# pratyushkumar211/industrial_nnmpc_2021

Measured on AMD Instinct MI355X. Metric: condensed-QP solves/sec (CDU offline datagen), higher is better.
Workload: dtype f64; 1 GPU; cdu_offline_data: synthetic CDU-size plant (n=4480 vars, m=8960 box rows, n_aug=284), 100000 sampled x0 per GPU per step, whole sequences u* written out; batch_per_gpu=100000, total_batch=100000, method=auto, parallelism=dp1 (sharded samples, 1 RCCL gather of the first moves pe...

## Files before the change

include/nnmpc.h:

```cpp
#ifndef NNMPC_H
#define NNMPC_H
#include <stdint.h>
#ifdef __cplusplus
extern "C" {
#endif

#define NNMPC_OK 0
#define NNMPC_EINVAL (-1)
#define NNMPC_EHIP (-2)
#define NNMPC_ENOMEM (-3)
#define NNMPC_ENOTIMPL (-4)

#define NNMPC_HOST 0
#define NNMPC_DEVICE 1

#define NNMPC_ST_OPTIMAL 0
#define NNMPC_ST_MAXITER 1
#define NNMPC_ST_NUMERIC 2

typedef struct nnmpc_qp nnmpc_qp;
typedef struct nnmpc_nn nnmpc_nn;

typedef struct {
  int32_t max_batch;
// ... 53 lines not shown
  double asm_predict_ms;
  double asm_predict_flops;
  int64_t asm_overlapped_passes;
  double mult_ms;
  int64_t mult_launches;
  double sens_ms;
  int64_t sens_launches;
  int64_t sens_lds_problems;
  int64_t sens_slab_problems;
  double sens_total_ms;
  double adj_ms;
  int64_t adj_launches;
  int64_t adj_lds_problems;
  int64_t adj_slab_problems;
  double adj_total_ms;
} nnmpc_qp_stats;

const char* nnmpc_last_error(void);

int nnmpc_qp_create(nnmpc_qp** out, int32_t n, int32_t nu, int32_t n_aug, const double* P,
                    const double* tq, const double* Kunc, const nnmpc_qp_opts* opts);
int nnmpc_qp_destroy(nnmpc_qp* h);

int nnmpc_qp_solve_batch(nnmpc_qp* h, int32_t B, const double* x0, const double* lb,
                         const double* ub, double* u, uint32_t* active, int32_t* status,
                         int32_t* iters, int32_t ptr_kind);

int nnmpc_qp_solve_batch_warm(nnmpc_qp* h, int32_t B, const double* x0, const double* lb,
                              const double* ub, const uint8_t* guess, double* u, uint32_t* active,
                              int32_t* status, int32_t* iters, int32_t ptr_kind);
// ... 214 lines not shown
```

industrial_nnmpc_2021_amd/_lib.py:

```python
import ctypes as C
import os

_HERE = os.path.dirname(os.path.abspath(__file__))
LIB_PATH = os.path.join(_HERE, "libnnmpc_hip.so")

HOST, DEVICE = 0, 1
ST_OPTIMAL, ST_MAXITER, ST_NUMERIC = 0, 1, 2
OUT_SEQUENCE, OUT_FIRST_MOVE = 0, 1
EINVAL, EHIP, ENOMEM, ENOTIMPL = -1, -2, -3, -4


class QpOpts(C.Structure):
    _fields_ = [("max_batch", C.c_int32), ("nb", C.c_int32), ("max_ipm_iters", C.c_int32),
                ("max_polish_rounds", C.c_int32), ("max_refine", C.c_int32),
                ("max_rounds", C.c_int32), ("sub_steps", C.c_int32), ("stale_max_changes", C.c_int32),
                ("stale_cg_limit", C.c_int32), ("method", C.c_int32), ("asm_max_active", C.c_int32),
                ("asm_max_rounds", C.c_int32), ("asm_f32_rounds", C.c_int32), ("seg_max", C.c_int32), ("asm_tail_batch", C.c_int32), ("asm_predict_iters", C.c_int32), ("asm_overlap", C.c_int32), ("ipm_tol", C.c_float), ("refine_tol", C.c_double),
                ("bound_tol", C.c_double)]


class QpStats(C.Structure):
    _fields_ = [("problems", C.c_int64), ("rounds", C.c_int64), ("factorizations", C.c_int64),
                ("ipm_iterations", C.c_int64), ("panel_launches", C.c_int64),
                ("panel_ms", C.c_double), ("diag_ms", C.c_double), ("trsv_ms", C.c_double),
                ("total_ms", C.c_double), ("panel_flops", C.c_double), ("trsv_solves", C.c_int64), ("asm_solved", C.c_int64),
                ("asm_rounds", C.c_int64), ("asm_gemm_launches", C.c_int64), ("asm_gemm_ms", C.c_double),
                ("asm_gemm_flops", C.c_double), ("asm_lambda_ms", C.c_double), ("asm_update_ms", C.c_double), ("asm_lambda_flops", C.c_double),
                ("asm_lambda_bytes", C.c_double), ("asm_e1max", C.c_double),
                ("asm_e2max", C.c_double), ("asm_full_checks", C.c_int64), ("asm_lambda32_ms", C.c_double),
                ("asm_lambda64_ms", C.c_double), ("asm_lambda32_flops", C.c_double),
                ("asm_lambda32_launches", C.c_int64), ("asm_lambda64_launches", C.c_int64), ("asm_far_passes", C.c_int64), ("asm_side_ms", C.c_double),
                ("asm_small_passes", C.c_int64), ("asm_predict_launches", C.c_int64), ("asm_predict_ms", C.c_double),
                ("asm_predict_flops", C.c_double), ("asm_overlapped_passes", C.c_int64),
                ("mult_ms", C.c_double), ("mult_launches", C.c_int64),
                ("sens_ms", C.c_double), ("sens_launches", C.c_int64), ("sens_lds_problems", C.c_int64),
                ("sens_slab_problems", C.c_int64), ("sens_total_ms", C.c_double),
                ("adj_ms", C.c_double), ("adj_launches", C.c_int64), ("adj_lds_problems", C.c_int64),
                ("adj_slab_problems", C.c_int64), ("adj_total_ms", C.c_double)]


CL_MPC, CL_NN, CL_SATDLQR, CL_US, CL_NN_UNSTD = 0, 1, 2, 3, 4
NN_STRUCTURED, NN_UNSTD, NN_UNSTD_RELU = 0, 1, 2
CL_PLANT_LINEAR, CL_PLANT_CSTRS_FLASH, CSTRS_NPAR = 0, 1, 51


class ClModel(C.Structure):
    _fields_ = [(k, C.c_int32) for k in ("nx", "nu", "ny", "nd", "nz")] + \
               [(k, C.c_void_p) for k in ("A", "B", "C", "Bp", "Aaug", "Baug", "Caug", "L", "tb", "Qb", "Qy", "q0", "Cd",
                                          "Eb", "Xb", "Xu", "Qaug", "Raug", "Maug", "ulb", "uub", "x0", "xhat0", "uprev0")]


class ClSlot(C.Structure):
    _fields_ = [("kind", C.c_int32), ("qp", C.c_void_p), ("nlayers", C.c_int32), ("dims", C.c_void_p), ("W", C.c_void_p),
# ... 308 lines not shown
```

industrial_nnmpc_2021_amd/csrc/qp_asm.h:

```cpp
#pragma once
#include <hip/hip_runtime.h>
#include <stdint.h>
#include <type_traits>

#if defined(ASM_WG_TU) && ASM_WG_TU >= 0
#define ASM_OWN_KERNELS 0
#else
#define ASM_OWN_KERNELS 1
#endif

namespace nnmpc {

constexpr int ASM_MLDS = 176;
constexpr int ASM_TS = 16 * 17;
enum { ASM_RUN = 0, ASM_DONE = 1, ASM_FALLBACK = 2, ASM_CERT = 3, ASM_WIDE = 4, ASM_INVALID = 5 };
constexpr int ASM_NBIN = 8;
constexpr int ASM_NREG = 6;
constexpr int ASM_NCNT = 40;
constexpr int ASM_CNT_KSUM = 0;
constexpr int ASM_CNT_SLAB = 1;
constexpr int ASM_CNT_ROWS64 = 2;
constexpr int ASM_CNT_LAST = 3;
constexpr int ASM_CNT_F64 = 4;
constexpr int ASM_CNT_F32 = 16;
// ... 5 lines not shown
constexpr int ASM_CNT_BIG64R = 31;
constexpr int ASM_CNT_BIG32B = 39;
constexpr double ASM_REFINE_TOL = 1e-12;
constexpr int ASM_GRACE = 10;
constexpr int ASM_CNT_WIDE = 12;
constexpr int ASM_CNT_WKSUM = 30;
constexpr int ASM_TAIL_MB = 8;
constexpr int ASM_CNT_TAIL = 35;
constexpr int ASM_CNT_FFTILES = 38;
constexpr int ASM_CNT_DONE = 14;
__host__ __device__ constexpr int asm_list_counter(int list) {
  return list < ASM_NBIN ? 4 + list : (list < ASM_NLIST ? ASM_CNT_F32 + list - ASM_NBIN : (list == ASM_NLIST ? ASM_CNT_BIG32 : (list == ASM_NLIST + 1 ? ASM_CNT_BIG64 : (list == ASM_NLIST + 2 ? ASM_CNT_BIG32B : ASM_CNT_BIG64R))));
}
__host__ __device__ constexpr int asm_list_of_counter(int c) { return c >= ASM_CNT_F32 ? ASM_NBIN + c - ASM_CNT_F32 : c - 4; }
constexpr int ASM_NKG = 3;
constexpr int ASM_NSCAN = ASM_NLIST + 9 + 2 * ASM_NKG;
constexpr int ASM_CNT_ROWS32 = 15;
__host__ __device__ constexpr int asm_bin_cap(int b) { return 16 * (b + 4); }

struct AsmDev {
  int n, np, nu, nseg;
  int max_active;
  int max_rounds;
  double bound_tol, stat_tol, pscale;
  double e1max, e2max;
  const double* x0;
  int ka;
  const double* Kunc;
  int pred_w;
  int pred_f64;
  int winit;
// ... 43 lines not shown
  unsigned char* redo;
  int* lrank;
  int* ctot;
  int use_f32;
  int W;
  int* rowprob;
  int wrows;
  unsigned char* wmark;
  const double* xhw;
  int tail_gi;
  int use_wg;
  int refine;
  double refine_tol;
  int refine_later;
  int early64;
  int* wflag;
  double* work;
  double* scratch;
  double* u_out;
  int ldu, nout;
  uint32_t* act_out;
  int* status_out;
  int* iters_out;
  int words;
};

__device__ __forceinline__ size_t tri(int i, int j) { return (size_t)i * (i + 1) / 2 + j; }

#if ASM_OWN_KERNELS
__global__ __launch_bounds__(256) void asm_init_k(AsmDev d, int nrows) {
// ... 15 lines not shown
      const double x = d.xunc[o + r];
      double lb = lbf, ub = ubf;
      if (!kfix) { const int k = r % d.nu; lb = d.lb[(size_t)p * d.nu + k]; ub = d.ub[(size_t)p * d.nu + k]; }
      s = x > ub ? 1 : (x < lb ? 2 : 0);
    }
    d.st[(size_t)p * d.n + r] = (unsigned char)s;
  }
  int invalid = 0;
  for (int k = lane; k < d.nu; k += 64) invalid |= !(d.lb[(size_t)p * d.nu + k] <= d.ub[(size_t)p * d.nu + k]);
  for (int k = lane; k < d.ka; k += 64) invalid |= !(fabs(d.x0[(size_t)p * d.ka + k]) <= 1.79e308);
  invalid = __any(invalid);
  if (lane == 0) {
    d.rounds[p] = 0; d.state[p] = invalid ? ASM_INVALID : ASM_RUN;
    d.prec[p] = (d.use_f32 && !d.guess && !(d.pred_w && d.pred_f64)) ? 0 : 1;
    d.redo[p] = 0;
    d.ninf_best[p] = 0x7fffffff; d.alpha[p] = ASM_GRACE;
    d.hi[p] = max(wi, d.guess ? 0 : d.pred_w);
  }
}
#endif

__device__ __forceinline__ int asm_count_one(const AsmDev& d, int p, int hi_p, int* wsum) {
  const int tid = threadIdx.x, lane = tid & 63, wave = tid >> 6;
  const unsigned char* st = d.st + (size_t)p * d.n;
  const bool words = (d.n & 3) == 0;
  const int hi = min(d.n, hi_p);
  const int nw = words ? (hi + 3) >> 2 : hi;
  const int per = (nw + 255) / 256;
  const int j0 = min(nw, tid * per), j1 = min(nw, j0 + per);
  const uint32_t* sw = reinterpret_cast<const uint32_t*>(st);
// ... 57 lines not shown
    int k = inc - c;
    if (words) {
      for (int j = j0; j < j1; ++j) {
        const uint32_t w = sw[j];
        if (w & 0xffu) idx[k++] = 4 * j;
        if (w & 0xff00u) idx[k++] = 4 * j + 1;
        if (w & 0xff0000u) idx[k++] = 4 * j + 2;
        if (w & 0xff000000u) idx[k++] = 4 * j + 3;
      }
    } else {
      for (int j = j0; j < j1; ++j) if (st[j]) idx[k++] = j;
    }
  }
  return m;
}
#if ASM_OWN_KERNELS
__global__ __launch_bounds__(256) void asm_count_k(AsmDev d) {
  const int p = blockIdx.x * 4 + (threadIdx.x >> 6);
  if (p >= d.nseg || d.state[p] != ASM_RUN) return;
  const int m = asm_count_wave(d, p, d.hi[p]);
  if ((threadIdx.x & 63) == 0) {
    d.mg[p] = m;
    if (m <= d.max_active && d.work) {
      const double md = (double)m;
      d.work[3 * p] += md * md * md / 3.0 + 2.0 * md * md;
      d.work[3 * p + 1] += 8.0 * (md * (md + 1.0) / 2.0 + 2.0 * md);
      if (d.prec[p] == 0 && m <= (d.use_wg ? ASM_BIG32B : ASM_BIG32)) d.work[3 * p + 2] += md * md * md / 3.0 + 2.0 * md * md;
    }
    if (m > d.max_active) d.state[p] = ASM_FALLBACK;
  }
}
#endif

constexpr int ASM_COL_ROW = 5 + ASM_NLIST;
constexpr int ASM_COL_WCNT = ASM_COL_ROW + 2 * ASM_NKG, ASM_COL_WK = ASM_COL_WCNT + 1;
constexpr int ASM_WG_SETS = 256;
__device__ __forceinline__ int asm_scan_col(const AsmDev& d, int p, bool& run) {
  run = p < d.nseg && d.state[p] == ASM_RUN;
  if (!run) return -1;
  const int m = d.mg[p];
  if (m > ASM_MLDS) return (d.prec[p] == 0 && m <= ASM_BIG32) ? 1 + ASM_NLIST : ((d.use_wg && m <= ASM_WG_SETS) ? 2 + ASM_NLIST : ((d.use_wg && d.prec[p] == 0 && m <= ASM_BIG32B) ? 3 + ASM_NLIST : ((d.use_wg && d.prec[p] == 1 && m <= ASM_BIG32B) ? 4 + ASM_NLIST : 0)));
  const int b = max((m + 15) / 16, 4) - 4;
  return 1 + (d.prec[p] == 0 ? ASM_NBIN + b : b);
}
__host__ __device__ inline int asm_kgroup_of(int kl, int kref, int nu) {
  const int st10 = 10 * (kl / nu), sref = kref / nu;
  return st10 <= 7 * sref ? 0 : (st10 <= 8 * sref ? 1 : 2);
}
__host__ __device__ inline int asm_kgroup_bound_of(int g, int kref, int nu) {
  const int sref = kref / nu;
  return ((g == 0 ? 7 : 8) * sref / 10 + 1) * nu - 1;
}
__device__ __forceinline__ int asm_kgroup(const AsmDev& d, int kl) { return asm_kgroup_of(kl, d.kref, d.nu); }
__device__ __forceinline__ int asm_kgroup_bound(const AsmDev& d, int g) { return asm_kgroup_bound_of(g, d.kref, d.nu); }
// ... 11 lines not shown
  const bool r32 = (col > ASM_NBIN + (d.refine ? ASM_NBIN : 0) && col <= 1 + ASM_NLIST) || col == 3 + ASM_NLIST;
  const int rcol = run ? ASM_COL_ROW + (r32 ? ASM_NKG : 0) + asm_kgroup(d, kl) : -1;
  int myrank = 0, myrow = 0;
#pragma unroll
  for (int c = 0; c < 2 * ASM_NKG; ++c) {
    const unsigned long long mk = __ballot(rcol == ASM_COL_ROW + c);
    if (rcol == ASM_COL_ROW + c) myrow = __popcll(mk & lt);
    if (lane == 0) wtot[ASM_COL_ROW + c][wave] = __popcll(mk);
  }
#pragma unroll
  for (int c = 0; c <= ASM_NLIST + 4; ++c) {
    const unsigned long long mk = __ballot(col == c);
    if (col == c) myrank = __popcll(mk & lt);
    if (lane == 0) wtot[c][wave] = __popcll(mk);
  }
  int km = kl, ks = run ? kl + 1 : 0;
  const bool wm = p < d.nseg && d.wmark[p] != 0;
  int wk = 0;
  if (wm) { const int m = d.mg[p]; wk = m > 0 ? d.idxg[(size_t)p * d.max_active + m - 1] + 1 : 1; }
  const unsigned long long wmk = __ballot(wm);
  for (int off = 32; off > 0; off >>= 1) { km = max(km, __shfl_xor(km, off)); ks += __shfl_xor(ks, off); wk += __shfl_xor(wk, off); }
  if (lane == 0) { wtot[ASM_NSCAN - 1][wave] = km; wtot[ASM_NSCAN - 2][wave] = ks; wtot[ASM_COL_WCNT][wave] = __popcll(wmk); wtot[ASM_COL_WK][wave] = wk; }
  __syncthreads();
  if (run) {
    for (int w = 0; w < wave; ++w) { myrow += wtot[rcol][w]; myrank += wtot[col][w]; }
    d.row[p] = myrow;
    d.lrank[p] = myrank;
  }
  if (tid < ASM_NSCAN) {
    int t = 0;
// ... 11 lines not shown
  if (tid < ASM_NSCAN) {
    int t = 0, all = 0;
    if (tid == ASM_NSCAN - 1) { for (int j = 0; j < (int)gridDim.x; ++j) t = max(t, d.ctot[(size_t)j * ASM_NSCAN + tid]); all = t; }
    else {
      for (int j = 0; j < (int)gridDim.x; ++j) { const int v = d.ctot[(size_t)j * ASM_NSCAN + tid]; if (j < (int)blockIdx.x) t += v; all += v; }
    }
    base[tid] = t; total[tid] = all;
  }
  __syncthreads();
  if (blockIdx.x == gridDim.x - 1 && tid < ASM_NSCAN) {
    if (tid == ASM_NSCAN - 1) {
      d.counters[3] = total[tid];
    } else if (tid == ASM_NSCAN - 2) d.counters[0] = total[tid];
    else if (tid == ASM_COL_WCNT) d.counters[ASM_CNT_WIDE + 1] = total[tid];
    else if (tid == ASM_COL_WK) d.counters[ASM_CNT_WKSUM] = total[tid];
    else if (tid == 0) d.counters[1] = total[0];
    else if (tid <= ASM_NLIST + 4) d.counters[asm_list_counter(tid - 1)] = total[tid];
    else if (tid == ASM_COL_ROW) { int t = 0; for (int g = 0; g < ASM_NKG; ++g) t += total[ASM_COL_ROW + g]; d.counters[2] = t; }
    else if (tid == ASM_COL_ROW + ASM_NKG) { int t = 0; for (int g = 0; g < ASM_NKG; ++g) t += total[ASM_COL_ROW + ASM_NKG + g]; d.counters[ASM_CNT_ROWS32] = t; }
  }
  if (p < d.nseg) d.wmark[p] = 0;
  bool run;
  const int col = asm_scan_col(d, p, run);
  if (!run) return;
  const int m = d.mg[p];
  const int kl = m > 0 ? d.idxg[(size_t)p * d.max_active + m - 1] : 0;
  const bool r32 = (col > ASM_NBIN + (d.refine ? ASM_NBIN : 0) && col <= 1 + ASM_NLIST) || col == 3 + ASM_NLIST;
  const int c0 = ASM_COL_ROW + (r32 ? ASM_NKG : 0), g = asm_kgroup(d, kl);
  int row = d.row[p] + base[c0 + g];
  for (int gg = 0; gg < g; ++gg) row += total[c0 + gg];
  d.row[p] = row;
  d.rowk[p] = r32;
  atomicMax(&d.kblk[(r32 ? d.nkblk / 2 : 0) + (row >> 6)], kl);
  const int pos = base[col] + d.lrank[p];
  if (col == 0) d.biglist[pos] = p;
  else d.binlist[(size_t)(col - 1) * d.nseg + pos] = p;
}
#endif

typedef double f64x4_t __attribute__((ext_vector_type(4)));
__device__ __forceinline__ double rdlane_d(double x, int l) {
  const int lo = __builtin_amdgcn_readlane(__double2loint(x), l);
  const int hi = __builtin_amdgcn_readlane(__double2hiint(x), l);
  return __hiloint2double(hi, lo);
}
__device__ __forceinline__ f64x4_t tile_mma_nt(const double* A, const double* B, int lane) {
  f64x4_t acc = {0.0, 0.0, 0.0, 0.0};
  const int li = lane & 15, kq = lane >> 4;
#pragma unroll
  for (int s = 0; s < 4; ++s)
// ... 615 lines not shown
  const int* idx = d.idxg + (size_t)p * d.max_active;
  const int m = __builtin_amdgcn_readfirstlane(d.mg[p]);
  if (m <= 0) return;
  ASM_STAMP(0);
  int* ix = reinterpret_cast<int*>(ys);
  for (int i = lane; i < MB * 16; i += 64) {
    const int a = idx[min(i, m - 1)], k = a % d.nu;
    ix[i] = a;
    const double v = d.xunc[o + a] - (st[a] == 1 ? d.ub[(size_t)p * d.nu + k] : d.lb[(size_t)p * d.nu + k]);
    rv[i] = i < m ? (T)v : T(0);
  }
  ASM_FENCE();
  T lam[MB];
  AsmRefine<MB> rf;
  const bool refine = N::F32 && d.rowk[p] == 0;
  if (N::F32) { rf.xunc = d.xunc + o; rf.lb = d.lb + (size_t)p * d.nu; rf.ub = d.ub + (size_t)p * d.nu; rf.st = st; rf.idx = idx; }
  const int bad = asm_reg_core<T, MB, asm_nl<T>(MB), false, N::F32>(d, m, ix, dt, Yt, ys, rv, lt, idt, lam, lane, wg, wave, rf, refine);
  if (N::F32 && refine && bad != 1) {
    if (bad == 2 && lane == 0) d.redo[p] = 2;
    double* lrow64 = d.lam + (size_t)d.row[p] * d.np;
#pragma unroll
    for (int I = 0; I < MB; ++I) {
      const int i = 16 * I + li;
      if (lq == 0 && i < m) lrow64[idx[i]] = bad == 2 ? rf.lam64[I] : (double)lam[I];
    }
    return;
  }
  if (bad) {
    if (lane == 0) { if (N::F32) { d.prec[p] = 1; d.redo[p] = 1; } else d.state[p] = ASM_FALLBACK; }
    return;
  }
  if (!N::F32 && lane == 0) d.prec[p] = 1;
// ... 200 lines not shown
}
#endif
constexpr int ASM_REG2_LDS = (2 * asm_rw<double>(11) + ASM_TS) * 8;
#if ASM_OWN_KERNELS
__global__ __launch_bounds__(128, 1) void asm_lambda_reg2_k(AsmDev d) {
  int w = blockIdx.x;
  {
    const int nb = (d.counters[4 + 7] + 1) >> 1;
    if (w < nb) { asm_lambda_reg<double, 11, 2>(d, 7, w); return; }
    w -= nb;
  }
  asm_lambda_reg<double, 10, 2>(d, 6, w);
  static_assert(ASM_NBIN == 8 && ASM_MLDS == 176, "classes 6 and 7 are the 10- and 11-block sets");
}
#endif
constexpr int ASM_REG32_LDS = (4 * asm_rw<float>(ASM_NREG + 3) + ASM_TS) * 4;
#if ASM_OWN_KERNELS
__global__ __launch_bounds__(256, 2) void asm_lambda_reg32_k(AsmDev d) {
  int w = blockIdx.x;
#define ASM_REG_CLASS(B)                                                            \
  {                                                                                 \
    const int nb = (d.counters[ASM_CNT_F32 + B] + 3) >> 2;                          \
    if (w < nb) { asm_lambda_reg<float, B + 4, 4>(d, ASM_NBIN + B, w); return; }    \
    w -= nb;                                                                        \
  }
  ASM_REG_CLASS(5) ASM_REG_CLASS(4) ASM_REG_CLASS(3) ASM_REG_CLASS(2) ASM_REG_CLASS(1) ASM_REG_CLASS(0)
#undef ASM_REG_CLASS
}
#endif

constexpr int ASM_REG32B_LDS = (4 * asm_rw<float>(11) + ASM_TS) * 4;
#if ASM_OWN_KERNELS
__global__ __launch_bounds__(256, 1) void asm_lambda_reg32b_k(AsmDev d) {
  int w = blockIdx.x;
  {
    const int nb = (d.counters[ASM_CNT_F32 + 7] + 3) >> 2;
    if (w < nb) { asm_lambda_reg<float, 11, 4>(d, ASM_NBIN + 7, w); return; }
    w -= nb;
  }
  asm_lambda_reg<float, 10, 4>(d, ASM_NBIN + 6, w);
}
#endif

}
#ifndef ASM_NO_WG_KERNELS
#include "qp_wg.h"
#endif
namespace nnmpc {

#if ASM_OWN_KERNELS
__global__ __launch_bounds__(256) void asm_update_k(AsmDev d) {
  const int lane = threadIdx.x & 63;
  const int p = blockIdx.x * 4 + (threadIdx.x >> 6);
  if (p >= d.nseg || d.state[p] != ASM_RUN) return;
  const int rdo = d.redo[p];
  if (rdo == 1) {
    if (lane == 0) d.redo[p] = 0;
    return;
  }
  if (rdo && lane == 0) d.redo[p] = 0;
  const bool f32_phase = d.rowk[p] != 0;
  const size_t o = (size_t)p * d.np, orow = (size_t)d.row[p] * d.np;
  unsigned char* st = d.st + (size_t)p * d.n;
  const int W = min(d.W, d.n);
  const int m = d.mg[p];
  const int* idx = d.idxg + (size_t)p * d.max_active;
  __shared__ unsigned short ch_r[4][8][64];
  __shared__ unsigned char ch_s[4][8][64];
  const int wv = threadIdx.x >> 6;
  int chg = 0, rmax = 0x7fffffff;
  double l1 = 0.0, lmin = 1e300;
  double res_r = 0.0, res_b = 0.0;
  auto scan = [&](int mode) {
    for (int r = lane; r < W; r += 64) {
      if (st[r]) continue;
      const int k = r % d.nu;
// ... 71 lines not shown
    sure = bnd <= d.stat_tol * d.pscale && lmin > bnd;
    for (int r = lane; r < d.n; r += 64) {
      const int k = r % d.nu, s = st[r];
      const double x = s == 0 ? d.xunc[o + r] - d.xh[orow + r]
                              : (s == 1 ? d.ub[(size_t)p * d.nu + k] : d.lb[(size_t)p * d.nu + k]);
      if (r < d.nout) d.u_out[(size_t)p * d.ldu + r] = x;
      if (!sure) d.x[o + r] = x;
    }
  }
  if (lane == 0) {
    const int rd = d.rounds[p] + 1;
    d.rounds[p] = rd;
    if (tot > 0 && d.hi[p] < W) d.hi[p] = W;
    const bool refine_next = d.refine_later && m <= ASM_MLDS;
    if (tot == 0 && !grade64 && !(f32_phase && refine_next)) d.prec[p] = 1;
    if (tot > 0 && tot <= d.early64 && f32_phase && !refine_next) d.prec[p] = 1;
    if (settle_wide) d.state[p] = ASM_WIDE;
    else if (settled) {
      d.state[p] = sure ? ASM_CERT : ASM_DONE;
      if (!sure) atomicAdd(&d.counters[ASM_CNT_DONE], 1);
    } else if (rd >= d.max_rounds) d.state[p] = ASM_FALLBACK;
  }
}
#endif

#if ASM_OWN_KERNELS
__global__ __launch_bounds__(256) void asm_wide_k(AsmDev d, int fused_c0) {
  const int lane = threadIdx.x & 63;
  const int w = blockIdx.x * 4 + (threadIdx.x >> 6);
  if (w >= d.wrows) return;
// ... 668 lines not shown
```

industrial_nnmpc_2021_amd/csrc/qp_solver.hip:

```cpp
#include <hip/hip_runtime.h>
#include <stdint.h>
#include <stdio.h>
#include <stdarg.h>
#include <string.h>
#include <vector>
#include <algorithm>
#include <cmath>
#include <cstdlib>
#include "../../include/nnmpc.h"
#define ASM_WG_TU (-1)
#include "chol_kernels.h"
#include "gemm_kernels.h"
#include "qp_asm.h"
#include "qp_wide.h"
#include "qp_small.h"
#include "qp_predict.h"
#include "qp_mult.h"
#include "qp_sens.h"
#include "qp_adj.h"
#include "dev_res.h"
static constexpr int ASM_SMALL9_LDS_MAX = 100 * 1024;

using namespace nnmpc;

// ... 595 lines not shown
  float* pdiag;
  double pscale;
  float* L;
  float* Y;
  float* Dacc;
  unsigned long long* trsv_count;
  QpDev d;
  bool have_inverse;
  double* H64;
  double* Kunc64;
  double *asm_xunc, *asm_x, *asm_scratch;
  int* asm_wflag;
  unsigned char* asm_wmark;
  unsigned char* asm_st;
  int *asm_state, *asm_rounds, *asm_biglist, *asm_status, *asm_binlist, *asm_idxg, *asm_mg, *asm_row, *asm_lrank, *asm_ctot;
  unsigned char *asm_prec, *asm_redo, *asm_alpha, *asm_rowk;
  float* H32;
  int *asm_ninf, *asm_hi;
  double tqmax;
  int asm_pool;
  double asm_e1max, asm_e2max;
  struct Far { int W, r, rp; double *U, *Vx, *Vl, *cu; int* kt; double ksum; double efar; };
  std::vector<Far> far;
  std::vector<int> far_missing;
  double p_inf = 0.0;
  struct AsmView {
    double *lam = nullptr, *xh = nullptr, *xhw = nullptr, *tnorm = nullptr, *tslack = nullptr;
    float *lam32 = nullptr, *xh32 = nullptr;
    int *rowprob = nullptr, *kblk = nullptr, *counters = nullptr;
    int rows = 0;
  };
// ... 17 lines not shown
  hipEvent_t ev_wfork = nullptr, ev_wide = nullptr;
  int* pin_cnt = nullptr;
  int* pin_st = nullptr;
  bool profiling;
  bool gemm_error = false;
  size_t ev_used;
  bool ev_failed = false;
  struct EvRec { int kind; hipEvent_t e0, e1; double flops; };
  std::vector<EvRec> ev_recs;
  nnmpc_qp_stats stats;
  enum {
         SC_U = 0, SC_ACT, SC_ST, SC_IT, SC_GUESS, SC_MULT, SC_X0, SC_LB, SC_UB, SC_FLAG,
         SC_FB_GUESS, SC_FB_LIST, SC_FB_X0, SC_FB_LB, SC_FB_UB, SC_FB_U, SC_FB_ACT, SC_FB_ST, SC_FB_IT,
         SC_S_CNT, SC_S_LIST, SC_S_XP, SC_S_T, SC_S_LAM, SC_S_X, SC_S_AREP, SC_S_SLAB,
         SC_A_KT,
         SC_COUNT };
  bool kunct_ok = false;
  DevRes res{SC_COUNT};
  int ldu, nout;
};

namespace {

struct AsmSwitches {
  bool no_fused_wide;
  bool no_lazy_xunc;
  bool no_farfield;
  bool no_small_gemm;
  bool trace;
  int tail_gi;
// ... 15 lines not shown
  w.no_fused_wide = env_set("NNMPC_NO_FUSED_WIDE"); w.no_lazy_xunc = env_set("NNMPC_NO_LAZY_XUNC"); w.no_farfield = env_set("NNMPC_NO_FARFIELD");
  w.no_small_gemm = env_set("NNMPC_NO_SMALL_GEMM"); w.trace = env_set("NNMPC_TRACE_ROUNDS");
  w.tail_gi = env_set("NNMPC_TAIL_GI") ? 1 : 0; w.use_wg = env_set("NNMPC_NO_WG") ? 0 : 1;
  w.refine = env_int("NNMPC_REFINE", 1); w.early64 = env_int("NNMPC_EARLY64", 4);
  { const char* e = getenv("NNMPC_REFINE_TOL"); w.refine_tol = e ? atof(e) : ASM_REFINE_TOL; }
  w.pred_iters = env_int("NNMPC_PRED_ITERS", -1); w.pred_wide = env_int("NNMPC_PRED_WIDE", -1); w.pred_f64 = env_int("NNMPC_PRED_F64", 0);
  w.pred_factor = env_int("NNMPC_PRED_FACTOR", 3); w.small_grace = env_int("NNMPC_SMALL_GRACE", ASM_SM_GRACE); w.tail_max = env_int("NNMPC_TAIL_MAX", 256);
  return w;
}
const AsmSwitches& asm_switches() {
  static const AsmSwitches w = read_switches();
  return w;
}
bool env_no_small() { return env_set("NNMPC_NO_SMALL"); }
bool env_overlap_off() { return env_int("NNMPC_OVERLAP", 1) == 0; }
long long env_overlap_rows(long long dflt) { const char* e = getenv("NNMPC_OVERLAP_ROWS"); return e ? std::max(0, atoi(e) / 128 * 128) : dflt; }

hipEvent_t ev_mark(nnmpc_qp* h, hipStream_t st) {
  hipEvent_t e = nullptr;
  if (h->res.pool_event(h->ev_used, &e)) { h->ev_failed = true; return nullptr; }
  ++h->ev_used;
  hipEventRecord(e, st);
  return e;
}
enum EvKind { EV_PANEL = 0, EV_DIAG, EV_TRSV, EV_TOTAL, EV_LAMBDA, EV_GEMM, EV_UPDATE, EV_LAMBDA32, EV_LAMBDA64, EV_SIDE, EV_PREDICT, EV_MULT, EV_SENS, EV_SENS_TOTAL, EV_ADJ, EV_ADJ_TOTAL };
struct EvScope {
  nnmpc_qp* h; int kind; double flops; hipEvent_t e0; hipStream_t st;
  EvScope(nnmpc_qp* h_, EvKind kind_, double flops_, hipStream_t st_ = nullptr) : h(h_), kind(kind_), flops(flops_), e0(nullptr), st(st_ ? st_ : h_->stream) {
    if (h->profiling) e0 = ev_mark(h, st);
  }
// ... 290 lines not shown
  if (wide) hipLaunchKernelGGL((asm_predict_k<8, 2>), dim3((nprob + 31) / 32), dim3(64 * PRED_NW), (pred_lds_bytes<8, 2>(h->nu)), s, a, pa);
  else if (nu4) hipLaunchKernelGGL((asm_predict_k<4, 4>), dim3((nprob + 63) / 64), dim3(64 * PRED_NW), (pred_lds_bytes<4, 4>(h->nu)), s, a, pa);
  else hipLaunchKernelGGL((asm_predict_k<4, 2, false>), dim3((nprob + 31) / 32), dim3(64 * PRED_NW), (pred_lds_bytes<4, 2>(h->nu)), s, a, pa);
  return 0;
}

struct WideStat { bool open; int view, far_rp, skip, cols; double far_ksum; };
struct AsmCall {
  nnmpc_qp* h; hipStream_t s; const AsmSwitches* sw;
  int nprob, segp;
  AsmDev a;
  int Wx, winit;
  bool lazy, small, tail_only;
  bool defer_cnt;
  bool overlap_on;
  int vW[2] = {0, 0}, vrows[2] = {0, 0};
  bool tail_ran[2] = {false, false};
  int pend = -1;
  WideStat wst = {false, 0, 0, 0, 0, 0.0}, wnext = wst;
  int fft_prev[2] = {0, 0};
  double pred_flops_per_it = 0.0;
  int kprev = 0;
};
struct PassLaunch { AsmDev ap; int fused_c0; bool inflight; };

void set_view(const nnmpc_qp* h, AsmDev& d, int v) {
  const nnmpc_qp::AsmView& V = h->view[v];
  d.lam = V.lam; d.xh = V.xh; d.xhw = V.xhw; d.T = V.xhw; d.tnorm = V.tnorm; d.tslack = V.tslack; d.lam32 = V.lam32; d.xh32 = V.xh32;
  d.rowprob = V.rowprob; d.kblk = V.kblk; d.counters = V.counters;
}
// ... 22 lines not shown
  a.ffU = a.ffVx = a.ffVl = a.ffcu = nullptr; a.ffk = nullptr; a.ffr = a.ffW = 0;
  a.ff_skip = 0; a.ff_err = 0.0; a.ff_efar = 0.0;
  set_view(h, a, 0);
  a.n = h->n; a.np = h->np; a.nu = h->nu; a.nseg = nprob;
  a.max_active = h->opts.asm_max_active; a.max_rounds = h->opts.asm_max_rounds;
  a.bound_tol = h->opts.bound_tol; a.stat_tol = 1e-8; a.pscale = h->pscale;
  a.e1max = h->asm_e1max; a.e2max = h->asm_e2max; a.x0 = h->x0_64; a.ka = h->ka;
  a.H = h->H64; a.lb = lb_dev; a.ub = ub_dev; a.xunc = h->asm_xunc; a.q64 = h->q64_all;
  a.x = h->asm_x; a.px = h->view[0].xh;
  a.st = h->asm_st; a.guess = guess_dev; a.state = h->asm_state; a.rounds = h->asm_rounds;
  a.biglist = h->asm_biglist; a.binlist = h->asm_binlist; a.idxg = h->asm_idxg; a.mg = h->asm_mg; a.row = h->asm_row; a.tqmax = h->tqmax; a.lrank = h->asm_lrank; a.ctot = h->asm_ctot; a.prec = h->asm_prec; a.redo = h->asm_redo; a.rowk = h->asm_rowk; a.H32 = h->H32; a.alpha = h->asm_alpha; a.ninf_best = h->asm_ninf; a.hi = h->asm_hi; a.nkblk = 2 * (h->seg_max / 64 + 2); a.kref = 0; a.use_f32 = h->opts.asm_f32_rounds >= 0; a.wrows = 0; a.wmark = h->asm_wmark; a.wflag = h->asm_wflag; a.W = h->np; a.scratch = h->asm_scratch; a.work = h->asm_work;
  a.u_out = u_dev; a.ldu = h->ldu; a.nout = h->nout; a.act_out = act_dev; a.status_out = h->asm_status; a.iters_out = it_dev; a.words = h->words;
  a.tail_gi = c.sw->tail_gi; a.use_wg = c.sw->use_wg;
  a.refine = 0; a.refine_later = c.sw->refine && a.use_f32; a.refine_tol = c.sw->refine_tol;
  a.early64 = c.sw->early64;
  a.pred_w = 0; a.pred_f64 = 0;
}

int first_sets(AsmCall& c) {
  nnmpc_qp* h = c.h;
  AsmDev& a = c.a;
  const int nprob = c.nprob;
  {
    const int env_it = c.sw->pred_iters;
    const int iters_req = env_it >= 0 ? (env_it == 0 ? -1 : std::min(env_it, (int)PRED_MAXIT)) : h->opts.asm_predict_iters;
    const int iters = iters_req == 0 ? (int)PRED_MAXIT : iters_req;
    if (iters > 0 && h->pred[0].L > 0.0 && !a.guess && !c.small && !c.tail_only && c.Wx >= PRED_W) {
      int wide = 0;
      if (h->pred[1].L > 0.0 && c.lazy) {
        if (c.sw->pred_wide >= 0) wide = c.sw->pred_wide;
// ... 12 lines not shown
      const int rc = launch_predictor(h, a, nprob, iters_req, wide, &W, &MR, &c.pred_flops_per_it);
      if (rc) return rc;
      a.pred_w = W;
      a.pred_f64 = c.sw->pred_f64;
    }
  }
  hipLaunchKernelGGL(asm_init_k, dim3((c.segp + 3) / 4), dim3(256), 0, c.s, a, c.segp);
  return 0;
}

std::vector<int> fetch_ints(const int* dev, int n) {
  std::vector<int> v(n);
  hipMemcpy(v.data(), dev, n * sizeof(int), hipMemcpyDeviceToHost);
  return v;
}
int trace_small(AsmCall& c) {
  nnmpc_qp* h = c.h;
  const int nprob = c.nprob;
  HIPCHK(stream_sync(c.s));
  const std::vector<int> rd = fetch_ints(h->asm_rounds, nprob), mg = fetch_ints(h->asm_mg, nprob), stt = fetch_ints(h->asm_state, nprob);
  long sum = 0, sm = 0, big = 0, bigit = 0, left = 0; int mx = 0, mm = 0, mxbig = 0, hist[8] = {0};
  for (int i = 0; i < nprob; ++i) {
    sum += rd[i]; mx = std::max(mx, rd[i]); sm += mg[i]; mm = std::max(mm, mg[i]); left += stt[i] == ASM_RUN;
    if (mg[i] > 32) { ++big; bigit += rd[i]; mxbig = std::max(mxbig, rd[i]); }
    hist[std::min(7, rd[i] / 8)]++;
  }
  fprintf(stderr, "asm small: %d problems, iterations mean %.2f max %d, final sets mean %.1f max %d; sets > 32: %ld (iterations mean %.1f max %d); handed on %ld; iterations/8 histogram",
          nprob, (double)sum / nprob, mx, (double)sm / nprob, mm, big, big ? (double)bigit / big : 0.0, mxbig, left);
  for (int b = 0; b < 8; ++b) fprintf(stderr, " %d", hist[b]);
  fprintf(stderr, "\n");
// ... 8 lines not shown
}
void trace_tail_only(AsmCall& c) {
  const int nprob = c.nprob;
  const std::vector<int> rd = fetch_ints(c.h->asm_rounds, nprob), mg = fetch_ints(c.h->asm_mg, nprob);
  long sum = 0, sm = 0; int mx = 0, mm = 0;
  for (int i = 0; i < nprob; ++i) { sum += rd[i]; mx = std::max(mx, rd[i]); sm += mg[i]; mm = std::max(mm, mg[i]); }
  fprintf(stderr, "asm tail only: %d problems, iterations mean %.2f max %d, active bounds mean %.1f max %d\n", nprob, (double)sum / nprob, mx, (double)sm / nprob, mm);
}
void trace_round(int rounds, bool inflight, const int* cnt) {
  fprintf(stderr, "asm round %d%s: fp64 %d f32 %d last-active %d wide-checked %d big %d big32 %d | fp64 classes", rounds, inflight ? " (beside the pass)" : "",
          cnt[ASM_CNT_ROWS64], cnt[ASM_CNT_ROWS32], cnt[ASM_CNT_LAST], cnt[ASM_CNT_WIDE + 1], cnt[ASM_CNT_SLAB], cnt[ASM_CNT_BIG32] + cnt[ASM_CNT_BIG32B]);
  for (int b = 0; b < ASM_NBIN; ++b) fprintf(stderr, " %d", cnt[ASM_CNT_F64 + b]);
  fprintf(stderr, " | f32 classes");
  for (int b = 0; b < ASM_NBIN; ++b) fprintf(stderr, " %d", cnt[ASM_CNT_F32 + b]);
  fprintf(stderr, "\n");
}
void trace_tail(AsmCall& c, int rounds, int nrun) {
  const std::vector<int> rd = fetch_ints(c.h->asm_rounds, c.nprob), bl = fetch_ints(c.h->asm_biglist, nrun);
  long sum = 0; int mx = 0;
  for (int i = 0; i < nrun; ++i) { const int r = rd[bl[i]] - rounds; sum += r; mx = std::max(mx, r); }
  fprintf(stderr, "asm tail after round %d: %d problems, iterations mean %.1f max %d\n", rounds, nrun, (double)sum / nrun, mx);
#ifdef ASM_TAIL_PROF
  unsigned long long tp[8];
  hipMemcpyFromSymbol(tp, HIP_SYMBOL(asm_tail_prof), sizeof tp);
  fprintf(stderr, "  tail clock sums (all workgroups): count/factor/solve %llu, substitutions %llu, x loop %llu, tests %llu, exchange %llu; iterations on the dense factor %llu, on a fresh factorisation %llu\n",
          tp[0], tp[1], tp[2], tp[3], tp[4], tp[5], tp[6]);
  memset(tp, 0, sizeof tp); hipMemcpyToSymbol(HIP_SYMBOL(asm_tail_prof), tp, sizeof tp);
#endif
}

// ... 192 lines not shown
      if (nwg32b) hipLaunchKernelGGL(asm_lambda_wg32b_k, dim3(nwg32b), dim3(512), (asm_wg_lds_bytes<float, ASM_WG_MB8>()), h->stream2, a);
      if (nwg32) hipLaunchKernelGGL(asm_lambda_wg32_k, dim3(nwg32), dim3(256), asm_wg_lds_bytes<float>(), h->stream2, a);
      if (cnt[ASM_CNT_BIG32] && !a.use_wg) hipLaunchKernelGGL(asm_lambda_tile32_k, dim3(std::min(cnt[ASM_CNT_BIG32], 4096)), dim3(512), ASM_TILE32_LDS, h->stream2, a);
      HIPCHK(hipEventRecord(h->ev_join, h->stream2));
    }
    if (side3) {
      HIPCHK(hipStreamWaitEvent(h->stream3, h->ev_fork, 0));
      EvScope e9(h, EV_SIDE, 0.0, h->stream3);
      if (nreg2_wg && a.use_wg) hipLaunchKernelGGL(asm_lambda_wg64s_k, dim3(cnt[ASM_CNT_F64 + 6] + cnt[ASM_CNT_F64 + 7]), dim3(128), asm_wg_lds_bytes<double>(), h->stream3, a);
      else if (nreg2_wg) hipLaunchKernelGGL(asm_lambda_reg2_k, dim3(nreg2_wg), dim3(128), ASM_REG2_LDS, h->stream3, a);
      if (nreg32b_wg) hipLaunchKernelGGL(asm_lambda_reg32b_k, dim3(nreg32b_wg), dim3(256), ASM_REG32B_LDS, h->stream3, a);
      HIPCHK(hipEventRecord(h->ev_join3, h->stream3));
    }
  }
  if (nreg_wg) { EvScope e8(h, EV_LAMBDA64, 0.0); hipLaunchKernelGGL(asm_lambda_reg_k, dim3(nreg_wg), dim3(256), ASM_REG_LDS, s, a); }
  if (nreg32_wg) { EvScope e7(h, EV_LAMBDA32, 0.0); hipLaunchKernelGGL(asm_lambda_reg32_k, dim3(nreg32_wg), dim3(256), ASM_REG32_LDS, s, a); }
  if (side2) HIPCHK(hipStreamWaitEvent(s, h->ev_join, 0));
  if (side3) HIPCHK(hipStreamWaitEvent(s, h->ev_join3, 0));
  if (side4) HIPCHK(hipStreamWaitEvent(s, h->ev_join4, 0));
  return 0;
}

int window_gemms_and_update(AsmCall& c, int rv, int n64, int n32, const int* cnt) {
  nnmpc_qp* h = c.h;
  hipStream_t s = c.s;
  const AsmDev& a = c.a;
  const int nprob = c.nprob;
  const nnmpc_qp::AsmView& V = h->view[rv];
  {
    EvScope es(h, EV_GEMM, 2.0 * a.W * (double)cnt[ASM_CNT_KSUM]);
// ... 106 lines not shown
  {
    EvScope es(h, EV_GEMM, 2.0 * c.Wx * (double)h->ka * nprob);
    gemm64(h, h->asm_xunc, h->np, h->x0_64, h->ka, h->Kunc64, h->ka, c.segp, c.Wx, h->ka);
  }
  asm_args(c, lb_dev, ub_dev, guess_dev, u_dev, act_dev, it_dev);
  if (!guess_dev) HIPCHK(hipMemsetAsync(h->asm_st, 0, (size_t)nprob * h->n, s));
  if (int rc = first_sets(c)) return rc;
  memset(h->pin_cnt, 0, 2 * ASM_NCNT * sizeof(int));
  HIPCHK(hipMemsetAsync(h->view[0].counters, 0, 2 * ASM_NCNT * sizeof(int), s));
  if (c.small)
    if (int rc = small_pass(c)) return rc;
  c.defer_cnt = c.tail_only && !sw.trace;
  if (c.tail_only)
    if (int rc = tail_only_pass(c)) return rc;
  c.overlap_on = h->opts.asm_overlap >= 0 && h->view[1].rows > 0 && !env_overlap_off();
  c.vW[0] = c.vW[1] = h->np;

  const int round_cap = 2 * a.max_rounds + 2;
  int rounds = 0;
  for (; !c.tail_only && rounds < round_cap; ++rounds) {
    const int pv = c.pend;
    PassLaunch pl = {a, -1, false};
    if (pv >= 0)
      if (int rc = launch_pass(c, pv, pl)) return rc;
    if (!a.pred_w) a.refine_later = 0;
    a.refine = a.refine_later && rounds >= 1;
    a.kref = c.kprev;
    int rv = pl.inflight ? 1 - pv : 0;
    int n64 = 0, n32 = 0, nrun = 0;
    const int* cnt = nullptr;
    for (bool recount = false;; recount = true) {
      if (int rc = count_round(c, rv, recount)) return rc;
      cnt = h->pin_cnt + rv * ASM_NCNT;
      n64 = cnt[ASM_CNT_ROWS64]; n32 = cnt[ASM_CNT_ROWS32]; nrun = n64 + n32;
      if (!pl.inflight || nrun <= h->view[rv].rows) break;
      if (int rc = finish_pass(c, pl)) return rc;
      rv = 0;
    }
    c.kprev = cnt[ASM_CNT_LAST];
    if (sw.trace) trace_round(rounds, pl.inflight, cnt);
    if (nrun == 0) {
// ... 2 lines not shown
      --rounds;
      continue;
    }
    if (nrun <= std::min(h->asm_pool, sw.tail_max) && (rounds >= (a.pred_w ? 2 : 6) || c.small)) {
      if (int rc = run_tail(c, rv, nrun, rounds, pl.inflight)) return rc;
      if (!pl.inflight) {
        rounds = 0;
        break;
      }
      a.Wx = c.Wx;
      if (int rc = finish_pass(c, pl)) return rc;
      h->stats.asm_overlapped_passes += 1;
      continue;
    }
    h->stats.asm_rounds += 1;
    a.W = std::min(h->np, ((cnt[ASM_CNT_LAST] + 1 + h->nu + 127) / 128) * 128);
    if (a.W > c.Wx) {
      EvScope es(h, EV_GEMM, 2.0 * (a.W - c.Wx) * (double)h->ka * nprob);
      extend_xunc(c, a.W, c.segp, false);
    }
    if (int rc = launch_multipliers(c, cnt, pl.inflight)) return rc;
    if (int rc = window_gemms_and_update(c, rv, n64, n32, cnt)) return rc;
    c.vW[rv] = a.W;
    c.vrows[rv] = a.W < h->n ? n64 : 0;
    c.pend = c.vrows[rv] ? rv : -1;
    if (pl.inflight) {
      if (int rc = finish_pass(c, pl)) return rc;
      h->stats.asm_overlapped_passes += 1;
    }
  }
  std::vector<int> fb;
  if (int rc = certify_and_collect(c, rounds >= round_cap, st_dev, fb)) return rc;
  return pdip_fallback(c, fb, x0_dev, st_dev);
}

int launch_mult(nnmpc_qp* h, int nprob, const double* x0_dev, const double* u_dev, const uint32_t* act_dev, const int32_t* st_dev,
// ... 114 lines not shown
  A_(h->q64_all, G * np); A_(h->uunc_all, G * np);
  A_(h->lb_d, G * nu); A_(h->ub_d, G * nu);
  A_(h->in_stage, G * n_aug);
  if (int rc = res.pinned_alloc(&h->pin_cnt, 2 * ASM_NCNT + 4)) return rc;
  if (int rc = res.pinned_alloc(&h->pin_st, G)) return rc;
  A_(d.lb64, (size_t)S * nu); A_(d.ub64, (size_t)S * nu);
  A_(d.slot_prob, S); A_(d.age, S); A_(d.next_prob, 1);
  h->asm_pool = h->seg_max >= 4096 ? (asm_switches().tail_max > 1024 ? 2048 : 1024) : 256;
  nnmpc_qp::AsmView& v0 = h->view[0];
  A_(h->H64, (size_t)np * np); A_(h->Kunc64, (size_t)np * ka); A_(h->H32, (size_t)np * np);
  A_(h->asm_xunc, G * np); A_(h->asm_x, G * np); A_(v0.lam, G * np); A_(v0.xh, G * np);
  A_(v0.xhw, (G + 256) * np); A_(v0.rowprob, G + 256); A_(h->asm_wflag, G); A_(h->asm_wmark, G);
  A_(v0.tnorm, G + 128 * (ASM_NKG + 1)); A_(v0.tslack, G + 128 * (ASM_NKG + 1));
  A_(h->asm_st, G * n); A_(h->asm_state, G); A_(h->asm_rounds, G); A_(v0.counters, 2 * ASM_NCNT);
  A_(h->asm_biglist, G); A_(h->asm_status, G); A_(h->asm_binlist, (size_t)(ASM_NLIST + 4) * G);
  A_(h->asm_idxg, G * o.asm_max_active); A_(h->asm_mg, G); A_(h->asm_row, G); A_(h->asm_lrank, G); A_(h->asm_ctot, ((G + 1023) / 1024) * ASM_NSCAN); A_(h->asm_prec, G); A_(h->asm_redo, G); A_(h->asm_rowk, G); A_(v0.lam32, G * np); A_(v0.xh32, G * np); A_(h->asm_alpha, G); A_(h->asm_ninf, G); A_(h->asm_hi, G); A_(v0.kblk, 2 * (G / 64 + 2)); A_(h->asm_work, 3 * G);
  v0.rows = (int)G;
  A_(h->asm_scratch, (size_t)h->asm_pool * ((size_t)(o.asm_max_active / 16) * (o.asm_max_active / 16 + 1) / 2 * ASM_TS));
  {
    long long R = env_overlap_rows(std::max<long long>(1024, ((long long)G / 32 + 127) / 128 * 128));
    R = std::min<long long>(R, (long long)G);
    if (o.asm_overlap >= 0 && R > 0) {
      nnmpc_qp::AsmView& v1 = h->view[1];
      const size_t Rr = (size_t)R;
      A_(v1.lam, Rr * np); A_(v1.xh, Rr * np); A_(v1.xhw, (Rr + 256) * np); A_(v1.lam32, Rr * np); A_(v1.xh32, Rr * np);
      A_(v1.tnorm, Rr + 128 * (ASM_NKG + 1)); A_(v1.tslack, Rr + 128 * (ASM_NKG + 1)); A_(v1.rowprob, Rr + 256); A_(v1.kblk, 2 * (G / 64 + 2));
      v1.counters = v0.counters + ASM_NCNT;
      v1.rows = (int)R;
    }
  }
#undef A_
// ... 786 lines not shown
```

Baseline: 7.804 million solves/s.

## Carry refined f64 multipliers from round zero to skip round-one re-solve

```diff
diff --git a/include/nnmpc.h b/include/nnmpc.h
--- a/include/nnmpc.h
+++ b/include/nnmpc.h
@@ -91,6 +91,7 @@
   int64_t adj_lds_problems;
   int64_t adj_slab_problems;
   double adj_total_ms;
+  int64_t asm_carried;
 } nnmpc_qp_stats;
 
 const char* nnmpc_last_error(void);
diff --git a/industrial_nnmpc_2021_amd/_lib.py b/industrial_nnmpc_2021_amd/_lib.py
--- a/industrial_nnmpc_2021_amd/_lib.py
+++ b/industrial_nnmpc_2021_amd/_lib.py
@@ -36,7 +36,8 @@
                 ("sens_ms", C.c_double), ("sens_launches", C.c_int64), ("sens_lds_problems", C.c_int64),
                 ("sens_slab_problems", C.c_int64), ("sens_total_ms", C.c_double),
                 ("adj_ms", C.c_double), ("adj_launches", C.c_int64), ("adj_lds_problems", C.c_int64),
-                ("adj_slab_problems", C.c_int64), ("adj_total_ms", C.c_double)]
+                ("adj_slab_problems", C.c_int64), ("adj_total_ms", C.c_double),
+                ("asm_carried", C.c_int64)]
 
 
 CL_MPC, CL_NN, CL_SATDLQR, CL_US, CL_NN_UNSTD = 0, 1, 2, 3, 4
diff --git a/industrial_nnmpc_2021_amd/csrc/qp_asm.h b/industrial_nnmpc_2021_amd/csrc/qp_asm.h
--- a/industrial_nnmpc_2021_amd/csrc/qp_asm.h
+++ b/industrial_nnmpc_2021_amd/csrc/qp_asm.h
@@ -43,7 +43,8 @@
 }
 __host__ __device__ constexpr int asm_list_of_counter(int c) { return c >= ASM_CNT_F32 ? ASM_NBIN + c - ASM_CNT_F32 : c - 4; }
 constexpr int ASM_NKG = 3;
-constexpr int ASM_NSCAN = ASM_NLIST + 9 + 2 * ASM_NKG;
+constexpr int ASM_NSCAN = ASM_NLIST + 10 + 2 * ASM_NKG;
+constexpr int ASM_CNT_CARRY = 24;
 constexpr int ASM_CNT_ROWS32 = 15;
 __host__ __device__ constexpr int asm_bin_cap(int b) { return 16 * (b + 4); }
 
@@ -117,6 +118,10 @@
   double refine_tol;
   int refine_later;
   int early64;
+  int carry;
+  double* stash;
+  unsigned char* cflag;
+  int* carrylist;
   int* wflag;
   double* work;
   double* scratch;
@@ -162,6 +167,7 @@
     d.rounds[p] = 0; d.state[p] = invalid ? ASM_INVALID : ASM_RUN;
     d.prec[p] = (d.use_f32 && !d.guess && !(d.pred_w && d.pred_f64)) ? 0 : 1;
     d.redo[p] = 0;
+    if (d.cflag) d.cflag[p] = 0;
     d.ninf_best[p] = 0x7fffffff; d.alpha[p] = ASM_GRACE;
     d.hi[p] = max(wi, d.guess ? 0 : d.pred_w);
   }
@@ -249,6 +255,7 @@
   }
   return m;
 }
+__device__ __forceinline__ bool asm_carried(const AsmDev& d, int p) { return d.carry == 2 && d.cflag[p] == 2; }
 #if ASM_OWN_KERNELS
 __global__ __launch_bounds__(256) void asm_count_k(AsmDev d) {
   const int p = blockIdx.x * 4 + (threadIdx.x >> 6);
@@ -256,7 +263,7 @@
   const int m = asm_count_wave(d, p, d.hi[p]);
   if ((threadIdx.x & 63) == 0) {
     d.mg[p] = m;
-    if (m <= d.max_active && d.work) {
+    if (m <= d.max_active && d.work && !asm_carried(d, p)) {
       const double md = (double)m;
       d.work[3 * p] += md * md * md / 3.0 + 2.0 * md * md;
       d.work[3 * p + 1] += 8.0 * (md * (md + 1.0) / 2.0 + 2.0 * md);
@@ -268,11 +275,13 @@
 #endif
 
 constexpr int ASM_COL_ROW = 5 + ASM_NLIST;
-constexpr int ASM_COL_WCNT = ASM_COL_ROW + 2 * ASM_NKG, ASM_COL_WK = ASM_COL_WCNT + 1;
+constexpr int ASM_COL_WCNT = ASM_COL_ROW + 2 * ASM_NKG, ASM_COL_WK = ASM_COL_WCNT + 1, ASM_COL_CARRY = ASM_COL_WK + 1;
+static_assert(ASM_COL_CARRY == ASM_NSCAN - 3, "the scan columns end with: carried, sum, max");
 constexpr int ASM_WG_SETS = 256;
 __device__ __forceinline__ int asm_scan_col(const AsmDev& d, int p, bool& run) {
   run = p < d.nseg && d.state[p] == ASM_RUN;
   if (!run) return -1;
+  if (asm_carried(d, p)) return ASM_COL_CARRY;
   const int m = d.mg[p];
   if (m > ASM_MLDS) return (d.prec[p] == 0 && m <= ASM_BIG32) ? 1 + ASM_NLIST : ((d.use_wg && m <= ASM_WG_SETS) ? 2 + ASM_NLIST : ((d.use_wg && d.prec[p] == 0 && m <= ASM_BIG32B) ? 3 + ASM_NLIST : ((d.use_wg && d.prec[p] == 1 && m <= ASM_BIG32B) ? 4 + ASM_NLIST : 0)));
   const int b = max((m + 15) / 16, 4) - 4;
@@ -314,6 +323,11 @@
     if (col == c) myrank = __popcll(mk & lt);
     if (lane == 0) wtot[c][wave] = __popcll(mk);
   }
+  {
+    const unsigned long long mk = __ballot(col == ASM_COL_CARRY);
+    if (col == ASM_COL_CARRY) myrank = __popcll(mk & lt);
+    if (lane == 0) wtot[ASM_COL_CARRY][wave] = __popcll(mk);
+  }
   int km = kl, ks = run ? kl + 1 : 0;
   const bool wm = p < d.nseg && d.wmark[p] != 0;
   int wk = 0;
@@ -355,6 +369,7 @@
     } else if (tid == ASM_NSCAN - 2) d.counters[0] = total[tid];
     else if (tid == ASM_COL_WCNT) d.counters[ASM_CNT_WIDE + 1] = total[tid];
     else if (tid == ASM_COL_WK) d.counters[ASM_CNT_WKSUM] = total[tid];
+    else if (tid == ASM_COL_CARRY) d.counters[ASM_CNT_CARRY] = total[tid];
     else if (tid == 0) d.counters[1] = total[0];
     else if (tid <= ASM_NLIST + 4) d.counters[asm_list_counter(tid - 1)] = total[tid];
     else if (tid == ASM_COL_ROW) { int t = 0; for (int g = 0; g < ASM_NKG; ++g) t += total[ASM_COL_ROW + g]; d.counters[2] = t; }
@@ -375,6 +390,7 @@
   atomicMax(&d.kblk[(r32 ? d.nkblk / 2 : 0) + (row >> 6)], kl);
   const int pos = base[col] + d.lrank[p];
   if (col == 0) d.biglist[pos] = p;
+  else if (col == ASM_COL_CARRY) d.carrylist[pos] = p;
   else d.binlist[(size_t)(col - 1) * d.nseg + pos] = p;
 }
 #endif
@@ -1020,8 +1036,19 @@
   T lam[MB];
   AsmRefine<MB> rf;
   const bool refine = N::F32 && d.rowk[p] == 0;
+  const bool keep = N::F32 && !refine && d.carry == 1;
   if (N::F32) { rf.xunc = d.xunc + o; rf.lb = d.lb + (size_t)p * d.nu; rf.ub = d.ub + (size_t)p * d.nu; rf.st = st; rf.idx = idx; }
-  const int bad = asm_reg_core<T, MB, asm_nl<T>(MB), false, N::F32>(d, m, ix, dt, Yt, ys, rv, lt, idt, lam, lane, wg, wave, rf, refine);
+  int bad = asm_reg_core<T, MB, asm_nl<T>(MB), false, N::F32>(d, m, ix, dt, Yt, ys, rv, lt, idt, lam, lane, wg, wave, rf, refine || keep);
+  if (N::F32 && keep && bad == 2) {
+    double* sp = d.stash + (size_t)p * ASM_MLDS;
+#pragma unroll
+    for (int I = 0; I < MB; ++I) {
+      const int i = 16 * I + li;
+      if (lq == 0 && i < m) sp[i] = rf.lam64[I];
+    }
+    if (lane == 0) d.cflag[p] = 1;
+    bad = 0;
+  }
   if (N::F32 && refine && bad != 1) {
     if (bad == 2 && lane == 0) d.redo[p] = 2;
     double* lrow64 = d.lam + (size_t)d.row[p] * d.np;
@@ -1252,6 +1279,18 @@
   static_assert(ASM_NBIN == 8 && ASM_MLDS == 176, "classes 6 and 7 are the 10- and 11-block sets");
 }
 #endif
+__device__ __forceinline__ void asm_carry_copy(const AsmDev& d, int wg) {
+  const int lane = threadIdx.x & 63;
+  const int it = wg * 4 + (threadIdx.x >> 6);
+  if (it >= d.counters[ASM_CNT_CARRY]) return;
+  const int p = d.carrylist[it];
+  const int m = min(d.mg[p], ASM_MLDS);
+  const int* idx = d.idxg + (size_t)p * d.max_active;
+  const double* sp = d.stash + (size_t)p * ASM_MLDS;
+  double* lrow = d.lam + (size_t)d.row[p] * d.np;
+  for (int i = lane; i < m; i += 64) lrow[idx[i]] = sp[i];
+  if (lane == 0) { d.redo[p] = 2; d.cflag[p] = 0; }
+}
 constexpr int ASM_REG32_LDS = (4 * asm_rw<float>(ASM_NREG + 3) + ASM_TS) * 4;
 #if ASM_OWN_KERNELS
 __global__ __launch_bounds__(256, 2) void asm_lambda_reg32_k(AsmDev d) {
@@ -1264,6 +1303,7 @@
   }
   ASM_REG_CLASS(5) ASM_REG_CLASS(4) ASM_REG_CLASS(3) ASM_REG_CLASS(2) ASM_REG_CLASS(1) ASM_REG_CLASS(0)
 #undef ASM_REG_CLASS
+  asm_carry_copy(d, w);
 }
 #endif
 
@@ -1293,11 +1333,12 @@
   if (p >= d.nseg || d.state[p] != ASM_RUN) return;
   const int rdo = d.redo[p];
   if (rdo == 1) {
-    if (lane == 0) d.redo[p] = 0;
+    if (lane == 0) { d.redo[p] = 0; if (d.cflag) d.cflag[p] = 0; }
     return;
   }
   if (rdo && lane == 0) d.redo[p] = 0;
   const bool f32_phase = d.rowk[p] != 0;
+  const bool kept = d.carry == 1 && d.cflag[p] == 1;
   const size_t o = (size_t)p * d.np, orow = (size_t)d.row[p] * d.np;
   unsigned char* st = d.st + (size_t)p * d.n;
   const int W = min(d.W, d.n);
@@ -1399,6 +1440,7 @@
     if (tot > 0 && d.hi[p] < W) d.hi[p] = W;
     const bool refine_next = d.refine_later && m <= ASM_MLDS;
     if (tot == 0 && !grade64 && !(f32_phase && refine_next)) d.prec[p] = 1;
+    if (kept) d.cflag[p] = (f32_phase && tot == 0 && refine_next) ? 2 : 0;
     if (tot > 0 && tot <= d.early64 && f32_phase && !refine_next) d.prec[p] = 1;
     if (settle_wide) d.state[p] = ASM_WIDE;
     else if (settled) {
diff --git a/industrial_nnmpc_2021_amd/csrc/qp_solver.hip b/industrial_nnmpc_2021_amd/csrc/qp_solver.hip
--- a/industrial_nnmpc_2021_amd/csrc/qp_solver.hip
+++ b/industrial_nnmpc_2021_amd/csrc/qp_solver.hip
@@ -633,7 +633,8 @@
   unsigned char* asm_wmark;
   unsigned char* asm_st;
   int *asm_state, *asm_rounds, *asm_biglist, *asm_status, *asm_binlist, *asm_idxg, *asm_mg, *asm_row, *asm_lrank, *asm_ctot;
-  unsigned char *asm_prec, *asm_redo, *asm_alpha, *asm_rowk;
+  unsigned char *asm_prec, *asm_redo, *asm_alpha, *asm_rowk, *asm_cflag;
+  int* asm_carrylist;
   float* H32;
   int *asm_ninf, *asm_hi;
   double tqmax;
@@ -681,6 +682,7 @@
          SC_FB_GUESS, SC_FB_LIST, SC_FB_X0, SC_FB_LB, SC_FB_UB, SC_FB_U, SC_FB_ACT, SC_FB_ST, SC_FB_IT,
          SC_S_CNT, SC_S_LIST, SC_S_XP, SC_S_T, SC_S_LAM, SC_S_X, SC_S_AREP, SC_S_SLAB,
          SC_A_KT,
+         SC_CARRY,
          SC_COUNT };
   bool kunct_ok = false;
   DevRes res{SC_COUNT};
@@ -726,6 +728,7 @@
 }
 bool env_no_small() { return env_set("NNMPC_NO_SMALL"); }
 bool env_overlap_off() { return env_int("NNMPC_OVERLAP", 1) == 0; }
+bool env_carry_off() { return env_int("NNMPC_CARRY", 1) == 0; }
 long long env_overlap_rows(long long dflt) { const char* e = getenv("NNMPC_OVERLAP_ROWS"); return e ? std::max(0, atoi(e) / 128 * 128) : dflt; }
 
 hipEvent_t ev_mark(nnmpc_qp* h, hipStream_t st) {
@@ -1046,6 +1049,7 @@
   bool lazy, small, tail_only;
   bool defer_cnt;
   bool overlap_on;
+  bool carry_on;
   int vW[2] = {0, 0}, vrows[2] = {0, 0};
   bool tail_ran[2] = {false, false};
   int pend = -1;
@@ -1098,6 +1102,7 @@
   a.tail_gi = c.sw->tail_gi; a.use_wg = c.sw->use_wg;
   a.refine = 0; a.refine_later = c.sw->refine && a.use_f32; a.refine_tol = c.sw->refine_tol;
   a.early64 = c.sw->early64;
+  a.carry = 0; a.stash = nullptr; a.cflag = h->asm_cflag; a.carrylist = h->asm_carrylist;
   a.pred_w = 0; a.pred_f64 = 0;
 }
 
@@ -1140,6 +1145,11 @@
   hipMemcpy(v.data(), dev, n * sizeof(int), hipMemcpyDeviceToHost);
   return v;
 }
+std::vector<unsigned char> fetch_bytes(const unsigned char* dev, int n) {
+  std::vector<unsigned char> v(n);
+  hipMemcpy(v.data(), dev, n, hipMemcpyDeviceToHost);
+  return v;
+}
 int trace_small(AsmCall& c) {
   nnmpc_qp* h = c.h;
   const int nprob = c.nprob;
@@ -1178,6 +1188,14 @@
   fprintf(stderr, " | f32 classes");
   for (int b = 0; b < ASM_NBIN; ++b) fprintf(stderr, " %d", cnt[ASM_CNT_F32 + b]);
   fprintf(stderr, "\n");
+}
+int trace_carry(AsmCall& c, int rounds, const int* cnt) {
+  HIPCHK(stream_sync(c.s));
+  const std::vector<unsigned char> fl = fetch_bytes(c.h->asm_cflag, c.nprob);
+  long kept = 0;
+  for (int i = 0; i < c.nprob; ++i) kept += fl[i] == 1;
+  fprintf(stderr, "asm round %d carry: corrected-and-stashed %ld, carried %d of %d\n", rounds, kept, cnt[ASM_CNT_CARRY], c.nprob);
+  return 0;
 }
 void trace_tail(AsmCall& c, int rounds, int nrun) {
   const std::vector<int> rd = fetch_ints(c.h->asm_rounds, c.nprob), bl = fetch_ints(c.h->asm_biglist, nrun);
@@ -1400,6 +1418,7 @@
     }
   }
   if (nreg_wg) { EvScope e8(h, EV_LAMBDA64, 0.0); hipLaunchKernelGGL(asm_lambda_reg_k, dim3(nreg_wg), dim3(256), ASM_REG_LDS, s, a); }
+  nreg32_wg += (cnt[ASM_CNT_CARRY] + 3) / 4;
   if (nreg32_wg) { EvScope e7(h, EV_LAMBDA32, 0.0); hipLaunchKernelGGL(asm_lambda_reg32_k, dim3(nreg32_wg), dim3(256), ASM_REG32_LDS, s, a); }
   if (side2) HIPCHK(hipStreamWaitEvent(s, h->ev_join, 0));
   if (side3) HIPCHK(hipStreamWaitEvent(s, h->ev_join3, 0));
@@ -1536,6 +1555,9 @@
   if (c.tail_only)
     if (int rc = tail_only_pass(c)) return rc;
   c.overlap_on = h->opts.asm_overlap >= 0 && h->view[1].rows > 0 && !env_overlap_off();
+  c.carry_on = a.refine_later && a.pred_w && !c.tail_only && !env_carry_off();
+  if (c.carry_on)
+    if (int rc = h->res.slot(nnmpc_qp::SC_CARRY, &a.stash, (size_t)h->seg_max * ASM_MLDS * sizeof(double))) return rc;
   c.vW[0] = c.vW[1] = h->np;
 
   const int round_cap = 2 * a.max_rounds + 2;
@@ -1547,6 +1569,7 @@
       if (int rc = launch_pass(c, pv, pl)) return rc;
     if (!a.pred_w) a.refine_later = 0;
     a.refine = a.refine_later && rounds >= 1;
+    a.carry = c.carry_on ? (rounds == 0 ? 1 : (rounds == 1 ? 2 : 0)) : 0;
     a.kref = c.kprev;
     int rv = pl.inflight ? 1 - pv : 0;
     int n64 = 0, n32 = 0, nrun = 0;
@@ -1579,12 +1602,15 @@
       continue;
     }
     h->stats.asm_rounds += 1;
+    h->stats.asm_carried += cnt[ASM_CNT_CARRY];
     a.W = std::min(h->np, ((cnt[ASM_CNT_LAST] + 1 + h->nu + 127) / 128) * 128);
     if (a.W > c.Wx) {
       EvScope es(h, EV_GEMM, 2.0 * (a.W - c.Wx) * (double)h->ka * nprob);
       extend_xunc(c, a.W, c.segp, false);
     }
     if (int rc = launch_multipliers(c, cnt, pl.inflight)) return rc;
+    if (sw.trace && a.carry)
+      if (int rc = trace_carry(c, rounds, cnt)) return rc;
     if (int rc = window_gemms_and_update(c, rv, n64, n32, cnt)) return rc;
     c.vW[rv] = a.W;
     c.vrows[rv] = a.W < h->n ? n64 : 0;
@@ -1729,7 +1755,7 @@
   A_(v0.tnorm, G + 128 * (ASM_NKG + 1)); A_(v0.tslack, G + 128 * (ASM_NKG + 1));
   A_(h->asm_st, G * n); A_(h->asm_state, G); A_(h->asm_rounds, G); A_(v0.counters, 2 * ASM_NCNT);
   A_(h->asm_biglist, G); A_(h->asm_status, G); A_(h->asm_binlist, (size_t)(ASM_NLIST + 4) * G);
-  A_(h->asm_idxg, G * o.asm_max_active); A_(h->asm_mg, G); A_(h->asm_row, G); A_(h->asm_lrank, G); A_(h->asm_ctot, ((G + 1023) / 1024) * ASM_NSCAN); A_(h->asm_prec, G); A_(h->asm_redo, G); A_(h->asm_rowk, G); A_(v0.lam32, G * np); A_(v0.xh32, G * np); A_(h->asm_alpha, G); A_(h->asm_ninf, G); A_(h->asm_hi, G); A_(v0.kblk, 2 * (G / 64 + 2)); A_(h->asm_work, 3 * G);
+  A_(h->asm_idxg, G * o.asm_max_active); A_(h->asm_mg, G); A_(h->asm_row, G); A_(h->asm_lrank, G); A_(h->asm_ctot, ((G + 1023) / 1024) * ASM_NSCAN); A_(h->asm_prec, G); A_(h->asm_redo, G); A_(h->asm_rowk, G); A_(h->asm_cflag, G); A_(h->asm_carrylist, G); A_(v0.lam32, G * np); A_(v0.xh32, G * np); A_(h->asm_alpha, G); A_(h->asm_ninf, G); A_(h->asm_hi, G); A_(v0.kblk, 2 * (G / 64 + 2)); A_(h->asm_work, 3 * G);
   v0.rows = (int)G;
   A_(h->asm_scratch, (size_t)h->asm_pool * ((size_t)(o.asm_max_active / 16) * (o.asm_max_active / 16 + 1) / 2 * ASM_TS));
   {
```

New measurement: 7.937 million solves/s (median of 6 runs). 1.7% higher.
